# bioinfo-biols/CIRI-long

Hardware: AMD Instinct MI355X
Metric: reads/s through CCS+SSW+BSJ (1/2/4/8 MI355X); % HBM roofline (higher is better)
Workload: dtype int16

## Files before the change

ciri_long_amd/csrc/clh_api.hip:

```cpp
#include <hip/hip_runtime.h>
#include <stdint.h>
#include <stdio.h>
#include <stdlib.h>
#include <string.h>

#include <algorithm>
#include <chrono>
#include <mutex>
#include <string>
#include <vector>

#include "../../include/ciri_long_hip.h"
#include "../../include/ssw_legacy.h"
#include "clh_device.h"

static thread_local std::string g_err;
static thread_local int g_code = CLH_E_ARG;
static int fail(int code, const std::string& m) { g_err = m; g_code = code; return code; }
#define HIPCHK(expr)                                                                         \
    do {                                                                                     \
        hipError_t e_ = (expr);                                                              \
        if (e_ != hipSuccess) return fail(CLH_E_HIP, std::string(#expr) + ": " + hipGetErrorString(e_)); \
    } while (0)

// ... 110 lines not shown
    {
        (void)hipSetDevice(ctx->device);
        if (ran) (void)hipStreamSynchronize(last_stream);
        for (void* b : blocks) ctx->release(b);
        for (hipEvent_t e : events) (void)hipEventDestroy(e);
    }
    void* alloc(size_t bytes)
    {
        void* p = ctx->alloc(bytes);
        if (p) blocks.push_back(p);
        return p;
    }
    void* upload(const void* host, size_t bytes)
    {
        void* p = alloc(bytes);
        return p && (bytes == 0 || hipMemcpy(p, host, bytes, hipMemcpyHostToDevice) == hipSuccess) ? p : nullptr;
    }
    void free_block(void* p)
    {
        auto it = std::find(blocks.begin(), blocks.end(), p);
        if (it == blocks.end()) return;
        blocks.erase(it);
        ctx->release(p);
    }
    hipError_t event(hipEvent_t* e, unsigned flags = hipEventDefault)
    {
        const hipError_t r = hipEventCreateWithFlags(e, flags);
        if (r == hipSuccess) events.push_back(*e);
        return r;
    }
};

struct SswSwitches {
    bool no_scan, no_scanw, no_slices, no_prefilter, no_lanes, no_pf2, no_tb_rows, no_guess, pf2_always;
    int pf2_share;
};

static SswSwitches ssw_switches()
{
    SswSwitches sw;
    sw.no_scan = getenv("CLH_NO_SCAN") != nullptr;
    sw.no_scanw = getenv("CLH_NO_SCANW") != nullptr;
    sw.no_slices = getenv("CLH_NO_SLICES") != nullptr;
    sw.no_prefilter = getenv("CLH_NO_PREFILTER") != nullptr;
    sw.no_lanes = getenv("CLH_NO_LANES") != nullptr;
    sw.no_pf2 = getenv("CLH_NO_PF2") != nullptr;
    sw.no_tb_rows = getenv("CLH_NO_TB_ROWS") != nullptr;
    sw.no_guess = getenv("CLH_NO_GUESS") != nullptr;
    sw.pf2_always = getenv("CLH_PF2_ALWAYS") != nullptr;
    const char* share = getenv("CLH_PF2_SHARE");
    sw.pf2_share = share ? std::max(1, atoi(share)) : 8;
    return sw;
}

struct clh_plan : clh_owned {
    using clh_owned::clh_owned;
    int n = 0;
    clh_ssw_opts opts;
    SswSwitches sw;
    clh::SswParams params;
    bool quirk = false, do_cigar = false;
    std::vector<clh::SswTask> tasks;
    struct Seg { int rv, begin, count; int64_t ws_off = 0; int ws_slot = 0, ws_wgs = 0; int lmax = 0; };
    void* d_seg_ctr = nullptr;
    std::vector<clh::ScanSlice> slices;
    void *d_slices = nullptr, *d_parts = nullptr;
    struct PfClass {
        bool on = false;
        int ntasks = 0, nwork = 0, bpl = 0, cap = 0;
        void *d_win = nullptr, *d_pieces = nullptr, *d_work = nullptr, *d_dmin = nullptr, *d_queue = nullptr, *d_out = nullptr, *d_ctl = nullptr,
             *d_bound = nullptr, *d_parts = nullptr, *d_q2 = nullptr;
        int ws_row0 = 0, ws_slot = 0, ws_wgs = 0;
        int64_t ws_dirs_off = 0;
        int64_t extent = 0;
        int64_t word_cols = 0, lane_insts = 0;
        hipEvent_t ev[2] = {nullptr, nullptr};
        bool timed = false;
    } pf[2];
    int n_rows = 0;
    std::vector<int32_t> slice_base;
    void* d_slice_base = nullptr;
    int n_all = 0;
    std::vector<Seg> segs;
    void *d_tasks = nullptr, *d_results = nullptr, *d_colmax = nullptr, *d_cigars = nullptr, *d_cigar_len = nullptr,
         *d_pool = nullptr, *d_pool_head = nullptr;
    size_t colmax_elems = 0, cigar_elems = 0, strip_bytes = 0;
    unsigned long long pool_bytes = 0;
    void* d_strips = nullptr;
    hipEvent_t done_ev = nullptr;
    bool profiling = false;
    int64_t refs_bytes = -1;
    std::vector<hipEvent_t> ev;
    std::vector<int32_t> w32_prefix;
    bool alpha = false;
    void* d_alpha_mat = nullptr;
    const void *run_reads = nullptr, *run_refs = nullptr;

    int64_t reserve_ws(size_t bytes, int wgs, int* slot)
    {
        *slot = (int)((bytes + 255) & ~(size_t)255);
        strip_bytes = (strip_bytes + 255) & ~(size_t)255;
        const int64_t off = (int64_t)strip_bytes;
        strip_bytes += (size_t)*slot * (size_t)wgs;
        return off;
    }
};

extern "C" void clh_plan_destroy(clh_plan* pl) { delete pl; }

static int alpha_class_for(int64_t L)
{
    for (int b = 0; b < clh::kNumAlphaBuckets - 1; ++b)
        if (L <= clh::kAlphaRows[b]) return clh::kRvAlpha - b;
    return clh::kRvAlpha - (clh::kNumAlphaBuckets - 1);
}

static int rv_class_for(int64_t L)
{
    const int64_t rows = (L + 15) / 16 * 16;
    for (int i = 0; i < clh::kNumRvClasses; ++i)
        if (128 * clh::kRvClasses[i] >= rows) return clh::kRvClasses[i];
    return clh::kRvStrips;
}

static bool scan_class_ok(int64_t L, const clh_ssw_opts* o, int max_match, int bias, const SswSwitches& sw)
{
    return !sw.no_scan && L <= 254 && o->score_size != 1 && (int64_t)max_match * L + bias < 255 && o->gap_extend >= 0 && o->gap_extend <= 16 && o->gap_open <= 255;
}
// ... 262 lines not shown
    }
    for (const auto& sg : pl->segs) {
        if (sg.rv != clh::kRvScanSliced || pl->pf[0].on) continue;
        for (int k = 0; k < sg.count; ++k) {
            clh::SswTask& t = pl->tasks[sg.begin + k];
            const int64_t R = t.ref_len;
            const auto [overlap, own] = slice_geom(t.read_len, R, mx, o->gap_extend, 0);
            t.dir_off = (int64_t)pl->slices.size();
            int ns = 0;
            for (int64_t b = 0; b < R; b += own, ++ns) {
                clh::ScanSlice sl;
                memset(&sl, 0, sizeof(sl));
                sl.task = k; sl.own_begin = (int32_t)b; sl.c_begin = (int32_t)std::max<int64_t>(0, b - overlap); sl.c_end = (int32_t)std::min<int64_t>(R, b + own);
                sl.part = (int32_t)pl->slices.size();
                pl->slices.push_back(sl);
            }
            t.pad = ns;
        }
    }

    pl->d_tasks = n_all > 0 ? pl->upload(pl->tasks.data(), sizeof(clh::SswTask) * (size_t)n_all) : pl->alloc(sizeof(clh::SswTask));
    pl->d_results = pl->alloc(sizeof(clh::SswResult) * (size_t)std::max(pl->n_rows, 1));
    pl->d_cigar_len = pl->alloc(sizeof(int32_t) * (size_t)std::max(n_all, 1));
    if (!pl->d_tasks || !pl->d_results || !pl->d_cigar_len) return oom();
    if (!pl->slice_base.empty() && !(pl->d_slice_base = pl->upload(pl->slice_base.data(), sizeof(int32_t) * pl->slice_base.size()))) return oom();
    if (o->want_score2 && !(pl->d_colmax = pl->alloc(sizeof(uint16_t) * std::max<size_t>(colmax, 1)))) return oom();
    if (pl->do_cigar) {
        pl->d_cigars = pl->alloc(sizeof(uint32_t) * std::max<size_t>(cig, 1));
        pl->d_pool = pl->alloc((size_t)pl->pool_bytes);
        pl->d_pool_head = pl->alloc(clh::tb_head_bytes(n_all));
        if (!pl->d_cigars || !pl->d_pool || !pl->d_pool_head) return oom();
    }
    if (pl->strip_bytes && !(pl->d_strips = pl->alloc(pl->strip_bytes))) return oom();
    if (!pl->slices.empty()) {
        pl->d_slices = pl->upload(pl->slices.data(), sizeof(clh::ScanSlice) * pl->slices.size());
        pl->d_parts = pl->alloc(sizeof(clh::ScanPart) * pl->slices.size());
        if (!pl->d_slices || !pl->d_parts) return oom();
    }
    return pl;
}

extern "C" clh_plan* clh_ssw_plan(clh_ctx* ctx, int32_t n, const int64_t* read_off, const int64_t* ref_off,
                                  const int32_t* mask_len, const clh_ssw_opts* o)
{
    if (!ref_off) { fail(CLH_E_ARG, "clh_ssw_plan: null argument"); return nullptr; }
    return ssw_plan_build(ctx, n, read_off, ref_off, nullptr, nullptr, nullptr, mask_len, o);
}

extern "C" clh_plan* clh_ssw_plan_windows(clh_ctx* ctx, int32_t n, const int64_t* read_off, const int64_t* win_off, const int32_t* win_len,
                                          const uint8_t* win_rc, const int32_t* mask_len, const clh_ssw_opts* o)
{
    if (!win_off || !win_len) { fail(CLH_E_ARG, "clh_ssw_plan_windows: null argument"); return nullptr; }
    return ssw_plan_build(ctx, n, read_off, nullptr, win_off, win_len, win_rc, mask_len, o);
}

struct clh_genome : clh_owned {
    using clh_owned::clh_owned;
    int64_t len = 0;
    void *d_codes = nullptr, *d_pre = nullptr;
    void* d_ascii = nullptr;
    void* d_sites = nullptr;
    int64_t n_sites[4] = {0, 0, 0, 0};
};

extern "C" void clh_genome_destroy(clh_genome* g) { delete g; }

// ... 101 lines not shown
        t.ctg_off = ctg_off[i]; t.ctg_len = ctg_len[i]; t.start = start[i]; t.end = end[i]; t.clip_base = clip_base[i]; t.host_mask = host_mask[i];
    }
    clh_ctx* ctx = g->ctx;
    HIPCHK(hipSetDevice(ctx->device));
    const size_t tb = sizeof(clh::SpliceTask) * (size_t)n, ob = sizeof(int32_t) * 8 * (size_t)n;
    void* d_t = ctx->alloc(tb); void* d_o = ctx->alloc(ob);
    clh::SpliceSites sites;
    int64_t at = 0;
    for (int k = 0; k < 4; ++k) { sites.pos[k] = (const int64_t*)g->d_sites + at; sites.n[k] = g->n_sites[k]; at += g->n_sites[k]; }
    int rc = 0;
    if (!d_t || !d_o) rc = fail(CLH_E_HIP, "out of device memory");
    if (!rc && (hipMemcpyAsync(d_t, tasks.data(), tb, hipMemcpyHostToDevice, ctx->stream) != hipSuccess ||
                clh::launch_splice_scan((const uint8_t*)g->d_codes, (const uint8_t*)g->d_ascii, (const clh::SpliceTask*)d_t, n, search_extra, shift_threshold, is_canonical & 3,
                                        sites, (int32_t*)d_o, ctx->stream) != hipSuccess ||
                hipMemcpyAsync(out, d_o, ob, hipMemcpyDeviceToHost, ctx->stream) != hipSuccess ||
                hipStreamSynchronize(ctx->stream) != hipSuccess))
        rc = fail(CLH_E_HIP, "splice-signal scan failed");
    if (rc) (void)hipStreamSynchronize(ctx->stream);
    ctx->release(d_t); ctx->release(d_o);
    return rc;
}

extern "C" int clh_ssw_run(clh_plan* pl, const void* d_reads, const void* d_refs, void* stream_)
{
    if (!pl || !d_reads || !d_refs) return fail(CLH_E_ARG, "clh_ssw_run: null argument");
    HIPCHK(hipSetDevice(pl->ctx->device));
    hipStream_t st = stream_ ? (hipStream_t)stream_ : pl->ctx->stream;
    clh::SswParams P = pl->params;
    P.reads = (const int8_t*)d_reads; P.refs = (const int8_t*)d_refs;
    P.results = (clh::SswResult*)pl->d_results;
    P.colmax = (uint16_t*)pl->d_colmax;
    P.cigars = (uint32_t*)pl->d_cigars; P.cigar_len = (int32_t*)pl->d_cigar_len; P.dirs = (uint8_t*)pl->d_strips;
    P.no_guess = pl->sw.no_guess;
    pl->run_reads = d_reads; pl->run_refs = d_refs;
    if (pl->profiling && pl->ev.empty()) {
        pl->ev.resize(pl->segs.size() * 2 + 4);
        for (auto& e : pl->ev) HIPCHK(pl->event(&e));
    }
    clh_ctx* c = pl->ctx;
    const bool tb = pl->do_cigar && pl->n > 0;
    const bool fan = !pl->profiling && pl->segs.size() > 1;
    const size_t eb = pl->segs.size() * 2;
    if (tb) HIPCHK(hipMemsetAsync(pl->d_pool_head, 0, 4 * 68, st));
    if (fan) {
        HIPCHK(hipEventRecord(c->fork_ev, st));
        for (int i = 0; i < 3; ++i) HIPCHK(hipStreamWaitEvent(c->side[i], c->fork_ev, 0));
    }
    std::vector<size_t> ord(pl->segs.size());
    for (size_t k = 0; k < ord.size(); ++k) ord[k] = k;
    std::sort(ord.begin(), ord.end(), [&](size_t x, size_t y) {
        auto weight = [](int rv) { return rv == clh::kRvStrips ? 1000 : (rv == clh::kRvScanWide ? 900 : (rv == clh::kRvScanWideSliced ? 800 : (rv == clh::kRvScanTr ? 700 : (clh::rv_is_alpha(rv) ? 600 + clh::kRvAlpha - rv : rv)))); };
        const int rx = weight(pl->segs[x].rv), ry = weight(pl->segs[y].rv);
        return rx > ry;
    });
    clh::SswParams PG = P;
    PG.tasks = (const clh::SswTask*)pl->d_tasks;
    uint8_t* const pool = (uint8_t*)pl->d_pool;
    unsigned long long* const head = (unsigned long long*)pl->d_pool_head;
    auto traceback = [&](int first, int count, int seg, hipStream_t ls) -> int {
        const int rvbig = 32;
        if (!pl->sw.no_tb_rows) {
            HIPCHK(clh::launch_traceback_rows(PG, first, count, pl->n_all, seg, pool, head, pl->pool_bytes, ls));
            HIPCHK(clh::launch_traceback_rows_wide(PG, first, count, pl->n_all, seg, pool, head, pl->pool_bytes, ls));
        } else HIPCHK(clh::launch_traceback_pool(0, PG, first, count, pl->n_all, seg, pool, head, pl->pool_bytes, ls));
        HIPCHK(clh::launch_traceback_pool(rvbig, PG, first, count, pl->n_all, seg, pool, head, pl->pool_bytes, ls));
        if (pl->w32_prefix[first + count] > pl->w32_prefix[first]) HIPCHK(clh::launch_traceback_w32(PG, first, count, pool, head, pl->pool_bytes, ls));
// ... 138 lines not shown
    if (pl->do_cigar && pl->n > 0) {
        HIPCHK(hipEventElapsedTime(&k1b_ms[0], pl->ev[2 * ns + 0], pl->ev[2 * ns + 1]));
        HIPCHK(hipEventElapsedTime(&k1b_ms[1], pl->ev[2 * ns + 2], pl->ev[2 * ns + 3]));
    }
    return ns;
}

extern "C" int clh_plan_traceback_counts(clh_plan* pl, int32_t* counts)
{
    if (!pl || !counts || !pl->ran) return fail(CLH_E_ARG, "clh_plan_traceback_counts: no run yet");
    counts[0] = counts[1] = 0;
    if (!pl->d_pool_head) return 0;
    HIPCHK(hipSetDevice(pl->ctx->device));
    HIPCHK(hipStreamSynchronize(pl->last_stream));
    int32_t w[64];
    HIPCHK(hipMemcpy(w, (const char*)pl->d_pool_head + 16, sizeof(w), hipMemcpyDeviceToHost));
    for (int k = 0; k < 32; ++k) { counts[0] += w[k]; counts[1] += w[32 + k]; }
    return 0;
}

extern "C" int clh_plan_prefilter_stats(clh_plan* pl, int64_t* out)
{
    if (!pl || !out) return fail(CLH_E_ARG, "clh_plan_prefilter_stats: null argument");
    for (int k = 0; k < 6; ++k) out[k] = 0;
    if (!pl->ran) return 0;
    HIPCHK(hipSetDevice(pl->ctx->device));
    HIPCHK(hipStreamSynchronize(pl->last_stream));
    for (const auto& f : pl->pf) {
        if (!f.on) continue;
        clh::PfCtl c;
        HIPCHK(hipMemcpy(&c, f.d_ctl, sizeof(c), hipMemcpyDeviceToHost));
        out[0] += f.ntasks; out[1] += c.n_pruned; out[2] += c.qcount; out[3] += (int64_t)c.cols_scanned; out[4] += (int64_t)c.cols_window; out[5] += c.n_stage2;
    }
    return 0;
}

extern "C" int clh_plan_prefilter_timing(clh_plan* pl, float* ms, int64_t* work)
{
    if (!pl || !ms || !work) return fail(CLH_E_ARG, "clh_plan_prefilter_timing: null argument");
    if (!pl->ran || !pl->profiling) return fail(CLH_E_ARG, "profiling was not enabled for the last run");
    HIPCHK(hipSetDevice(pl->ctx->device));
    HIPCHK(hipStreamSynchronize(pl->last_stream));
    for (int ci = 0; ci < 2; ++ci) {
        const auto& f = pl->pf[ci];
        ms[ci] = 0.f; work[2 * ci] = work[2 * ci + 1] = 0;
        if (!f.on || !f.timed) continue;
        HIPCHK(hipEventElapsedTime(&ms[ci], f.ev[0], f.ev[1]));
        work[2 * ci] = f.word_cols; work[2 * ci + 1] = f.lane_insts;
    }
    return 0;
}

extern "C" const void* clh_ssw_results_dev(const clh_plan* pl) { return pl ? pl->d_results : nullptr; }

__global__ void cigar_gather_kernel(const uint32_t* __restrict__ src, const int32_t* __restrict__ src_off, const int64_t* __restrict__ dst_off,
                                    const int32_t* __restrict__ len, uint32_t* __restrict__ dst)
{
    const int a = blockIdx.x, L = len[a];
    const uint32_t* s = src + src_off[a];
    uint32_t* d = dst + dst_off[a];
    for (int k = threadIdx.x; k < L; k += blockDim.x) d[k] = s[k];
}

static int alpha_pool_rounds(clh_plan* pl, std::vector<clh::SswResult>& res)
{
    const int n = pl->n;
// ... 1285 lines not shown
```

ciri_long_amd/csrc/clh_device.h:

```cpp
#pragma once
#include <hip/hip_runtime.h>
#include <stdint.h>

namespace clh {

enum {
    CLH_STATUS_WORD = 1,
    CLH_STATUS_OVERFLOW8 = 2,
    CLH_STATUS_TRACE_ERR = 4,
    CLH_STATUS_NO_CIGAR = 8,
    CLH_STATUS_CIGAR_TRUNC = 16,
    CLH_STATUS_NEED_BIG = 32,
    CLH_STATUS_BAD_CODE = 64,
    CLH_STATUS_NEED_W32 = 128,
    CLH_STATUS_NEED_POOL = 256
};

struct SswTask {
    int64_t read_off;
    int64_t ref_off;
    int64_t colmax_off;
    int64_t dir_off;
    int32_t read_len;
    int32_t ref_len;
// ... 56 lines not shown
struct SswParams {
    const int8_t* reads;
    const int8_t* refs;
    const SswTask* tasks;
    SswResult* results;
    uint16_t* colmax;
    uint32_t* cigars;
    int32_t* cigar_len;
    uint8_t* dirs;
    int8_t mat[32];
    int32_t n, gapO, gapE, bias, max_match, score_size, flag, filters, filterd;
    int32_t null_code;
    const ScanSlice* slices;
    ScanPart* parts;
    int32_t n_real;
    const int32_t* slice_base;
    const PfWin* pf_win;
    const PfTask* pf_tasks;
    const PfWork* pf_work;
    uint8_t* pf_dmin;
    ScanSlice* pf_slices;
    PfOut* pf_out;
    PfCtl* pf_ctl;
    int32_t pf_bpl, pf_cap;
    int32_t* pf_q2;
    int32_t pf2_always;
    int32_t pf2_share;
    uint16_t* ws_bound;
    WsTask* ws_tasks;
    int32_t ws_row0;
    int32_t ws_slot_bytes;
    int64_t ws_dirs_off;
    int32_t no_guess;
};

static constexpr int CCS_SEG_CAP = 65;

struct CcsScan {
    int32_t period;
    int32_t ncuts;
    int32_t support;
    int32_t cuts[64];
};

struct CcsResult {
    int32_t nseg;
    int32_t ccs_len;
    int32_t period;
    int32_t status;
};

struct PoaScores {
    int32_t algorithm;
    int32_t m, n, g, e, q, c;
    int32_t min_cov;
};

struct CcsParams {
    const int8_t* reads;
    const int64_t* read_off;
    CcsScan* scan;
    CcsResult* results;
    int32_t* segs;
    int8_t* ccs;
    uint8_t* poa_ws;
    int* work_counter;
// ... 168 lines not shown
```

ciri_long_amd/csrc/ssw_scan.hip:

```cpp
#include <hip/hip_runtime.h>
#include <stdint.h>
#include "clh_device.h"
#include "clh_device_ops.h"

namespace clh {

namespace {



#ifndef SCAN_WAVES
#define SCAN_WAVES 3
#endif
static constexpr int SCAN_MAX_ROWS = 256;
static constexpr int SCAN_CPR_MAX = 8;
static constexpr int SCAN_PROF_WORDS = 6 * SCAN_CPR_MAX * 64;

struct ScanIn {
    const int8_t* read;
    int rstep;
    int L;
    int rows;
    const int8_t* ref;
    int cstep;
    int comp;
    int ncols;
    int terminate;
    uint16_t* colmax;
    int own0;
    int col_base;
};
struct ScanOut { int max, col, row; };

struct ScanLds {
    uint32_t* prof;
    const int* mat;
    short* bH;
    short* bE;
};

template <int CPR, bool GEQ>
__device__ void scan_chunk(const ScanIn& in, const ScanLds& lds, const int c0, const int parity, const bool first, const bool more,
                           const int gapO, const int gapE, int& best_score, int& best_col, int& best_row, int& tcol)
{
    constexpr int VEC = CPR < 4 ? CPR : 4;
    constexpr int NCH = CPR / VEC;
    const int lane = threadIdx.x & 63;
    const int K = CPR * gapE;
    const int kLo = 2 * lane * K;
    const uint32_t gO2 = dup16(gapO), gE2 = dup16(gapE);

    {
        int rlo[CPR], rhi[CPR];
#pragma unroll
        for (int t = 0; t < CPR; ++t) {
            const int jlo = c0 + 2 * CPR * lane + t, jhi = jlo + CPR;
            const int blo = jlo < in.ncols ? (int)in.ref[(int64_t)jlo * in.cstep] : 0, bhi = jhi < in.ncols ? (int)in.ref[(int64_t)jhi * in.cstep] : 0;
            rlo[t] = jlo < in.ncols ? ref_code(blo, in.comp) : 5;
            rhi[t] = jhi < in.ncols ? ref_code(bhi, in.comp) : 5;
        }
#pragma unroll
        for (int q = 0; q < 6; ++q)
#pragma unroll
            for (int t = 0; t < CPR; ++t) {
                const int slo = lds.mat[rlo[t] * 8 + q], shi = lds.mat[rhi[t] * 8 + q];
                lds.prof[((q * NCH + t / VEC) * 64 + lane) * VEC + (t % VEC)] = (uint32_t)(slo & 0xffff) | ((uint32_t)shi << 16);
            }
    }
    const short* bHin = lds.bH + (parity ^ 1) * SCAN_MAX_ROWS;
    const short* bEin = lds.bE + (parity ^ 1) * SCAN_MAX_ROWS;
    short* bHout = lds.bH + parity * SCAN_MAX_ROWS;
// ... 136 lines not shown
    res.score1 = fw.max;
    if (fw.max == 0) { res.ref_end1 = -1; res.read_end1 = 0; }
    else { res.ref_end1 = fw.col; res.read_end1 = fw.row; }
    if (task.mask_len >= 15 && colmax) { __syncthreads(); __builtin_amdgcn_fence(__ATOMIC_ACQUIRE, "agent"); second_best(colmax, refLen, res.ref_end1, task.mask_len, 0, res.score2, res.ref_end2); }
    else { res.score2 = 0; res.ref_end2 = task.mask_len >= 15 ? 0 : -1; }

    res.read_begin1 = -1;
    const bool want_begin = !(p.flag == 0 || (p.flag == 2 && res.score1 < p.filters));
    if (want_begin) {
        ScanIn rv;
        rv.L = res.read_end1 + 1; rv.rows = ((rv.L + 15) / 16) * 16; rv.read = read + res.read_end1; rv.rstep = -1;
        rv.ncols = res.ref_end1 + 1; rv.ref = ref + (int64_t)res.ref_end1 * rdir; rv.cstep = -rdir; rv.comp = task.ref_rc;
        rv.terminate = res.score1; rv.colmax = nullptr; rv.own0 = 0; rv.col_base = 0;
        const ScanOut r = scan_pass<GEQ>(rv, lds, p.gapO, p.gapE);
        if (r.max == 0) { res.ref_begin1 = -1; res.read_begin1 = res.read_end1; }
        else { res.ref_begin1 = res.ref_end1 - r.col; res.read_begin1 = res.read_end1 - r.row; }
    }
    if (lane == 0) p.results[task.out_index] = res;
}

template <bool GEQ>
__device__ ScanOut scan_forward(const SswParams& p, const SswTask& task, const ScanLds& lds, int c_begin, int own_begin, int c_end)
{
    const int rdir = task.ref_rc ? -1 : 1;
    uint16_t* colmax = p.colmax ? p.colmax + task.colmax_off : nullptr;
    ScanIn in;
    in.read = p.reads + task.read_off; in.rstep = 1; in.L = task.read_len;
    in.ref = p.refs + task.ref_off + (int64_t)c_begin * rdir; in.cstep = rdir; in.comp = task.ref_rc; in.ncols = c_end - c_begin;
    in.terminate = 1 << 30; in.colmax = colmax; in.own0 = own_begin - c_begin; in.col_base = c_begin;
    in.rows = colmax ? ((in.L + 15) / 16) * 16 : in.L;
    return scan_pass<GEQ>(in, lds, p.gapO, p.gapE);
}

#define SCAN_LDS_SETUP \
    __shared__ __attribute__((aligned(16))) uint32_t s_prof[SCAN_PROF_WORDS]; \
    __shared__ int s_mat[48]; \
    __shared__ short s_bH[2 * SCAN_MAX_ROWS], s_bE[2 * SCAN_MAX_ROWS]; \
    { const int lane_ = threadIdx.x & 63; \
      if (lane_ < 48) { const int b_ = lane_ >> 3, q_ = lane_ & 7; s_mat[lane_] = (b_ < p.n && q_ < p.n) ? (int)p.mat[b_ * p.n + q_] : 0; } } \
    __syncthreads(); \
    ScanLds lds; lds.prof = s_prof; lds.mat = s_mat; lds.bH = s_bH; lds.bE = s_bE;

}

template <bool GEQ>
__global__ void __launch_bounds__(64, SCAN_WAVES) ssw_scan_kernel(const SswParams p)
{
    SCAN_LDS_SETUP
    const SswTask task = p.tasks[blockIdx.x];
    const ScanOut fw = scan_forward<GEQ>(p, task, lds, 0, 0, task.ref_len);
    scan_finish<GEQ>(p, task, fw, lds);
}

template <bool GEQ>
__global__ void __launch_bounds__(64, SCAN_WAVES) ssw_scan_slice_kernel(const SswParams p)
{
    SCAN_LDS_SETUP
    const ScanSlice sl = p.slices[blockIdx.x];
    const SswTask task = p.tasks[sl.task];
    const ScanOut fw = scan_forward<GEQ>(p, task, lds, sl.c_begin, sl.own_begin, sl.c_end);
    if ((threadIdx.x & 63) == 0) { ScanPart pt; pt.max = fw.max; pt.col = fw.col; pt.row = fw.row; pt.pad = 0; p.parts[sl.part] = pt; }
}

template <bool GEQ>
__global__ void __launch_bounds__(64, SCAN_WAVES) ssw_scan_finish_kernel(const SswParams p)
{
    SCAN_LDS_SETUP
    const int lane = threadIdx.x & 63;
    const SswTask task = p.tasks[blockIdx.x];
    const int first = (int)task.dir_off, ns = task.pad;
    int v = 0, c = 0x7fffffff, r = 0;
    if (lane < ns) { const ScanPart pt = p.parts[first + lane]; v = pt.max; c = pt.max > 0 ? pt.col : 0x7fffffff; r = pt.row; }
#pragma unroll
    for (int d = 1; d < 64; d <<= 1) {
        const int v2 = __shfl_xor(v, d), c2 = __shfl_xor(c, d), r2 = __shfl_xor(r, d);
        const bool take = v2 > v || (v2 == v && c2 < c);
        v = take ? v2 : v; c = take ? c2 : c; r = take ? r2 : r;
    }
    ScanOut fw; fw.max = v; fw.col = v > 0 ? c : -1; fw.row = v > 0 ? r : 0;
    scan_finish<GEQ>(p, task, fw, lds);
}

template <bool GEQ>
// ... 249 lines not shown
```

ciri_long_amd/hip.py:

```python
import ctypes as C
import os
import sys

import numpy as np

_HERE = os.path.dirname(os.path.abspath(__file__))
SO_PATH = os.environ.get('CLH_LIB') or os.path.join(_HERE, 'libclh.so')


class HipUnavailable(RuntimeError):
    pass


class ClhError(RuntimeError):
    pass


class AlignRow(C.Structure):
    _fields_ = [('score1', C.c_uint16), ('score2', C.c_uint16), ('ref_begin1', C.c_int32), ('ref_end1', C.c_int32),
                ('read_begin1', C.c_int32), ('read_end1', C.c_int32), ('ref_end2', C.c_int32),
                ('cigar_off', C.c_int32), ('cigar_len', C.c_int32), ('status', C.c_int32)]


ALIGN_DTYPE = np.dtype([('score1', '<u2'), ('score2', '<u2'), ('ref_begin1', '<i4'), ('ref_end1', '<i4'),
# ... 92 lines not shown
        L.clh_edit_distance_batch.restype = C.c_int
        L.clh_edit_matrix_plan_create.restype = C.c_void_p
        L.clh_edit_matrix_plan_create.argtypes = [C.c_void_p, C.c_int32, C.c_void_p, C.c_void_p, C.c_int32, C.c_void_p, C.c_int32]
        L.clh_edit_matrix_plan_destroy.restype = None
        L.clh_edit_matrix_plan_destroy.argtypes = [C.c_void_p]
        L.clh_edit_matrix_plan_run.argtypes = [C.c_void_p, C.c_void_p]
        L.clh_edit_matrix_plan_sizes.argtypes = [C.c_void_p, C.POINTER(C.c_int64), C.POINTER(C.c_int64)]
        L.clh_edit_matrix_plan_fetch.argtypes = [C.c_void_p, C.c_void_p, C.c_int64, C.c_void_p, C.c_void_p, C.c_int64]
        L.clh_edit_matrix_plan_timing.argtypes = [C.c_void_p, C.c_void_p]
        L.clh_edit_matrix_batch.argtypes = [C.c_void_p, C.c_int32, C.c_void_p, C.c_void_p, C.c_int32, C.c_void_p, C.c_int32, C.c_void_p, C.c_int64,
                                            C.c_void_p, C.c_void_p, C.c_int64]
        L.clh_edit_align_plan_create.restype = C.c_void_p
        L.clh_edit_align_plan_create.argtypes = [C.c_void_p, C.c_int32, C.c_void_p, C.c_void_p, C.c_void_p, C.c_void_p, C.POINTER(EditAlignOpts)]
        L.clh_edit_align_plan_destroy.restype = None
        L.clh_edit_align_plan_destroy.argtypes = [C.c_void_p]
        L.clh_edit_align_plan_run.argtypes = [C.c_void_p, C.c_void_p]
        L.clh_edit_align_plan_fetch.argtypes = [C.c_void_p, C.c_void_p, C.c_void_p, C.c_int64, C.POINTER(C.c_int64), C.c_void_p, C.c_int64,
                                                C.POINTER(C.c_int64)]
        L.clh_edit_align_plan_timing.argtypes = [C.c_void_p, C.c_void_p]
        L.clh_edit_align_plan_caps.argtypes = [C.c_void_p, C.POINTER(C.c_int64), C.POINTER(C.c_int64)]
        L.clh_edit_align_batch.argtypes = [C.c_void_p, C.c_int32, C.c_void_p, C.c_void_p, C.c_void_p, C.c_void_p, C.POINTER(EditAlignOpts),
                                           C.c_void_p, C.c_void_p, C.c_int64, C.POINTER(C.c_int64), C.c_void_p, C.c_int64, C.POINTER(C.c_int64)]
        L.clh_poa_batch.argtypes = [C.c_void_p, C.c_int32, C.c_void_p, C.c_void_p, C.c_void_p, C.c_void_p, C.c_void_p, C.c_void_p,
                                    C.c_void_p, C.c_void_p, C.c_void_p]
        L.clh_ccs_results_dev.argtypes = [C.c_void_p, C.c_void_p, C.c_void_p, C.c_void_p]
        L.clh_ccs_plan_info.argtypes = [C.c_void_p, C.c_void_p]
        L.clh_ccs_plan_stats.argtypes = [C.c_void_p, C.c_void_p]
        L.clh_poa_last_stats.argtypes = [C.c_void_p, C.c_void_p]
        L.clh_plan_set_profiling.argtypes = [C.c_void_p, C.c_int]
        L.clh_plan_segments.argtypes = [C.c_void_p, C.c_int32, C.c_void_p, C.c_void_p, C.c_void_p, C.c_void_p]
        L.clh_plan_timing.argtypes = [C.c_void_p, C.c_int32, C.c_void_p, C.c_void_p]
        L.clh_plan_traceback_counts.argtypes = [C.c_void_p, C.c_void_p]
        L.clh_plan_prefilter_stats.argtypes = [C.c_void_p, C.c_void_p]
        L.clh_plan_prefilter_timing.argtypes = [C.c_void_p, C.c_void_p, C.c_void_p]
        L.clh_plan_set_refs_bytes.argtypes = [C.c_void_p, C.c_int64]
        _lib = L
    return _lib


def fastx_index(in_path, is_fastq, every=4096):
    n = C.c_int64(0); no = C.c_int64(0)
    L = lib()
    L.clh_fastx_index.argtypes = [C.c_char_p, C.c_int, C.c_int64, C.c_void_p, C.c_void_p, C.c_int64, C.c_void_p]
    cap = max(16, os.path.getsize(in_path) // max(1, 20 * every) + 16)
    off = np.zeros(cap, dtype=np.int64)
    if L.clh_fastx_index(os.fsencode(in_path), int(bool(is_fastq)), int(every), C.byref(n), off.ctypes.data, cap, C.byref(no)) != 0:
        raise ClhError('clh_fastx_index failed for %s' % in_path)
    return int(n.value), [int(x) for x in off[:no.value]]


def fastx_count(in_path, is_fastq):
    n = C.c_int64(0)
    if lib().clh_fastx_count(os.fsencode(in_path), int(bool(is_fastq)), C.byref(n)) != 0:
        raise ClhError('clh_fastx_count failed for %s' % in_path)
    return int(n.value)


def last_error():
    return lib().clh_last_error().decode()


def _check(rc, what):
    if rc != 0:
        raise ClhError('%s failed (%d): %s' % (what, rc, last_error()))


# ... 534 lines not shown
    def run(self, d_reads_ptr, d_refs_ptr, stream=0):
        _check(lib().clh_ssw_run(self._h, C.c_void_p(d_reads_ptr), C.c_void_p(d_refs_ptr), C.c_void_p(stream)), 'clh_ssw_run')

    def fetch(self):
        out = np.zeros(self.n, dtype=ALIGN_DTYPE)
        cap = int(2 * (self.read_off[-1] if self.n else 0) + 2 * self.n + 8) if self.want_cigar else 1
        cig = np.empty(cap, dtype=np.uint32)
        used = C.c_int64(0)
        _check(lib().clh_ssw_fetch(self._h, out.ctypes.data, cig.ctypes.data if self.want_cigar else None, cap, C.byref(used)), 'clh_ssw_fetch')
        return out, cig[:used.value]

    def set_refs_bytes(self, nbytes):
        lib().clh_plan_set_refs_bytes(self._h, int(nbytes))

    def set_profiling(self, on=True):
        lib().clh_plan_set_profiling(self._h, 1 if on else 0)

    def segments(self):
        rv = np.zeros(32, dtype=np.int32); cnt = np.zeros(32, dtype=np.int32)
        rb = np.zeros(32, dtype=np.int64); fb = np.zeros(32, dtype=np.int64)
        ns = lib().clh_plan_segments(self._h, 32, rv.ctypes.data, cnt.ctypes.data, rb.ctypes.data, fb.ctypes.data)
        return [(int(rv[k]), int(cnt[k]), int(rb[k]), int(fb[k])) for k in range(ns)]

    def traceback_counts(self):
        c = np.zeros(2, dtype=np.int32)
        _check(lib().clh_plan_traceback_counts(self._h, c.ctypes.data), 'clh_plan_traceback_counts')
        return int(c[0]), int(c[1])

    def prefilter_stats(self):
        c = np.zeros(6, dtype=np.int64)
        _check(lib().clh_plan_prefilter_stats(self._h, c.ctypes.data), 'clh_plan_prefilter_stats')
        return dict(zip(('alignments', 'pruned', 'slices', 'cols_computed', 'cols_window', 'second_stage'), (int(x) for x in c)))

    def prefilter_timing(self):
        ms = np.zeros(2, dtype=np.float32); w = np.zeros(4, dtype=np.int64)
        _check(lib().clh_plan_prefilter_timing(self._h, ms.ctypes.data, w.ctypes.data), 'clh_plan_prefilter_timing')
        return [(float(ms[k]), int(w[2 * k]), int(w[2 * k + 1])) for k in range(2)]

    def timing(self):
        a = np.zeros(32, dtype=np.float32); b = np.zeros(2, dtype=np.float32)
        ns = lib().clh_plan_timing(self._h, 32, a.ctypes.data, b.ctypes.data)
        if ns < 0:
            _check(ns, 'clh_plan_timing')
        return [float(a[k]) for k in range(ns)], (float(b[0]), float(b[1]))

    def results_dev_ptr(self):
        return lib().clh_ssw_results_dev(self._h)


class CcsPlan(_Handle):
    _destroy = 'clh_ccs_plan_destroy'

    def __init__(self, ctx, read_off):
        _Handle.__init__(self, ctx)
        self.read_off = np.ascontiguousarray(read_off, dtype=np.int64)
        self.n = len(self.read_off) - 1
        self._h = lib().clh_ccs_plan_create(ctx._h, self.n, self.read_off.ctypes.data)
        if not self._h:
            raise ClhError('clh_ccs_plan_create failed: %s' % last_error())

    def run(self, d_reads_ptr, stream=0):
        _check(lib().clh_ccs_run(self._h, C.c_void_p(d_reads_ptr), C.c_void_p(stream)), 'clh_ccs_run')

    def timing(self):
        ms = np.zeros(2, dtype=np.float32)
        _check(lib().clh_ccs_plan_timing(self._h, ms.ctypes.data), 'clh_ccs_plan_timing')
# ... 35 lines not shown
```

include/ciri_long_hip.h:

```cpp
#ifndef CIRI_LONG_HIP_H
#define CIRI_LONG_HIP_H

#include <stdint.h>

#ifdef __cplusplus
extern "C" {
#endif
#pragma GCC visibility push(default)

#define CLH_E_HIP        (-1)
#define CLH_E_ARG        (-2)
#define CLH_E_UNSUPPORTED (-3)
#define CLH_E_CAPACITY   (-4)

#define CLH_ST_WORD        1
#define CLH_ST_NULL        2
#define CLH_ST_TRACE_ERR   4
#define CLH_ST_NO_CIGAR    8
#define CLH_ST_CIGAR_TRUNC 16

typedef struct {
    uint16_t score1;
    uint16_t score2;
    int32_t ref_begin1;
// ... 7 lines not shown
} clh_align_t;

typedef struct clh_ctx clh_ctx;
typedef struct clh_plan clh_plan;

int clh_device_count(void);
const char* clh_last_error(void);
const char* clh_version(void);

clh_ctx* clh_create(int device);
void clh_destroy(clh_ctx* ctx);
int clh_device_of(const clh_ctx* ctx);

typedef struct {
    const int8_t* mat;
    int32_t n_mat;
    uint8_t gap_open;
    uint8_t gap_extend;
    uint8_t flag;
    int8_t score_size;
    uint16_t filters;
    int32_t filterd;
    int32_t want_score2;
    int32_t want_cigar;
} clh_ssw_opts;

clh_plan* clh_ssw_plan(clh_ctx* ctx, int32_t n, const int64_t* read_off, const int64_t* ref_off,
                       const int32_t* mask_len, const clh_ssw_opts* opts);
void clh_plan_destroy(clh_plan* plan);

int clh_plan_traceback_counts(clh_plan* pl, int32_t* counts);

int clh_plan_prefilter_stats(clh_plan* pl, int64_t* out);

int clh_plan_prefilter_timing(clh_plan* pl, float* ms, int64_t* work);

int clh_ssw_run(clh_plan* plan, const void* d_reads, const void* d_refs, void* stream);

int clh_plan_set_refs_bytes(clh_plan* plan, int64_t nbytes);

int clh_ssw_fetch(clh_plan* plan, clh_align_t* out, uint32_t* cigar_buf, int64_t cigar_cap, int64_t* cigar_used);

const void* clh_ssw_results_dev(const clh_plan* plan);

int clh_plan_set_profiling(clh_plan* plan, int on);
int clh_plan_segments(const clh_plan* plan, int32_t cap, int32_t* rv, int32_t* count, int64_t* read_bases, int64_t* ref_bases);
int clh_plan_timing(clh_plan* plan, int32_t cap, float* k1_ms, float* k1b_ms);

int clh_ssw_batch(clh_ctx* ctx, int32_t n, const int8_t* reads, const int64_t* read_off, const int8_t* refs,
                  const int64_t* ref_off, const int32_t* mask_len, const clh_ssw_opts* opts,
                  clh_align_t* out, uint32_t* cigar_buf, int64_t cigar_cap, int64_t* cigar_used);

#define CLH_CCS_SEG_CAP 65
typedef struct {
    int32_t nseg;
    int32_t ccs_len;
    int32_t period;
    int32_t status;
} clh_ccs_t;
typedef struct clh_ccs_plan clh_ccs_plan;
clh_ccs_plan* clh_ccs_plan_create(clh_ctx* ctx, int32_t n, const int64_t* read_off);
void clh_ccs_plan_destroy(clh_ccs_plan* plan);
int clh_ccs_run(clh_ccs_plan* plan, const void* d_reads, void* stream);
int clh_ccs_fetch(clh_ccs_plan* plan, clh_ccs_t* out, int32_t* segs, int8_t* ccs);
int clh_ccs_results_dev(const clh_ccs_plan* plan, const void** rows, const void** segs, const void** ccs);
int clh_ccs_plan_info(clh_ccs_plan* plan, int64_t* out);
// ... 89 lines not shown
```

Baseline: 5.235 million.

## Prune SSW scan columns with bit-parallel edit-distance lower bounds

```diff
diff --git a/ciri_long_amd/csrc/clh_api.hip b/ciri_long_amd/csrc/clh_api.hip
--- a/ciri_long_amd/csrc/clh_api.hip
+++ b/ciri_long_amd/csrc/clh_api.hip
@@ -166,8 +166,8 @@
 };
 
 struct SswSwitches {
-    bool no_scan, no_scanw, no_slices, no_prefilter, no_lanes, no_pf2, no_tb_rows, no_guess, pf2_always;
-    int pf2_share;
+    bool no_scan, no_scanw, no_slices, no_prefilter, no_lanes, no_pf2, no_tb_rows, no_guess, pf2_always, no_scan_prune;
+    int pf2_share, scan_prune_mult, scan_prune_share;
 };
 
 static SswSwitches ssw_switches()
@@ -184,6 +184,11 @@
     sw.pf2_always = getenv("CLH_PF2_ALWAYS") != nullptr;
     const char* share = getenv("CLH_PF2_SHARE");
     sw.pf2_share = share ? std::max(1, atoi(share)) : 8;
+    sw.no_scan_prune = getenv("CLH_NO_SCAN_PRUNE") != nullptr;
+    const char* mult = getenv("CLH_SCAN_PRUNE_MULT");
+    sw.scan_prune_mult = mult ? std::max(1, atoi(mult)) : 4;
+    const char* pshare = getenv("CLH_SCAN_PRUNE_SHARE");
+    sw.scan_prune_share = pshare ? std::min(100, std::max(0, atoi(pshare))) : 50;
     return sw;
 }
 
@@ -228,6 +233,7 @@
     std::vector<int32_t> w32_prefix;
     bool alpha = false;
     void* d_alpha_mat = nullptr;
+    void* d_scan_prune = nullptr;
     const void *run_reads = nullptr, *run_refs = nullptr;
 
     int64_t reserve_ws(size_t bytes, int wgs, int* slot)
@@ -556,6 +562,11 @@
         if (!pl->d_cigars || !pl->d_pool || !pl->d_pool_head) return oom();
     }
     if (pl->strip_bytes && !(pl->d_strips = pl->alloc(pl->strip_bytes))) return oom();
+    if (!alpha && !sw.no_scan_prune && prefilter_ok(o, mx, sw) &&
+        std::any_of(pl->segs.begin(), pl->segs.end(), [](const clh_plan::Seg& g) { return g.rv == clh::kRvScan; })) {
+        const unsigned long long zero[3] = {0, 0, 0};
+        if (!(pl->d_scan_prune = pl->upload(zero, sizeof(zero)))) return oom();
+    }
     if (!pl->slices.empty()) {
         pl->d_slices = pl->upload(pl->slices.data(), sizeof(clh::ScanSlice) * pl->slices.size());
         pl->d_parts = pl->alloc(sizeof(clh::ScanPart) * pl->slices.size());
@@ -723,6 +734,8 @@
     P.colmax = (uint16_t*)pl->d_colmax;
     P.cigars = (uint32_t*)pl->d_cigars; P.cigar_len = (int32_t*)pl->d_cigar_len; P.dirs = (uint8_t*)pl->d_strips;
     P.no_guess = pl->sw.no_guess;
+    P.scan_prune_ctr = (unsigned long long*)pl->d_scan_prune;
+    P.scan_prune = pl->d_scan_prune != nullptr; P.scan_prune_mult = pl->sw.scan_prune_mult; P.scan_prune_share = pl->sw.scan_prune_share;
     pl->run_reads = d_reads; pl->run_refs = d_refs;
     if (pl->profiling && pl->ev.empty()) {
         pl->ev.resize(pl->segs.size() * 2 + 4);
@@ -927,6 +940,17 @@
         HIPCHK(hipMemcpy(&c, f.d_ctl, sizeof(c), hipMemcpyDeviceToHost));
         out[0] += f.ntasks; out[1] += c.n_pruned; out[2] += c.qcount; out[3] += (int64_t)c.cols_scanned; out[4] += (int64_t)c.cols_window; out[5] += c.n_stage2;
     }
+    return 0;
+}
+
+extern "C" int clh_plan_scan_prune_stats(clh_plan* pl, int64_t* out)
+{
+    if (!pl || !out) return fail(CLH_E_ARG, "clh_plan_scan_prune_stats: null argument");
+    for (int k = 0; k < 3; ++k) out[k] = 0;
+    if (!pl->d_scan_prune) return 0;
+    HIPCHK(hipSetDevice(pl->ctx->device));
+    if (pl->ran) HIPCHK(hipStreamSynchronize(pl->last_stream));
+    HIPCHK(hipMemcpy(out, pl->d_scan_prune, 3 * sizeof(int64_t), hipMemcpyDeviceToHost));
     return 0;
 }
 
diff --git a/ciri_long_amd/csrc/clh_device.h b/ciri_long_amd/csrc/clh_device.h
--- a/ciri_long_amd/csrc/clh_device.h
+++ b/ciri_long_amd/csrc/clh_device.h
@@ -112,6 +112,10 @@
     int32_t ws_slot_bytes;
     int64_t ws_dirs_off;
     int32_t no_guess;
+    int32_t scan_prune;
+    int32_t scan_prune_mult;
+    int32_t scan_prune_share;
+    unsigned long long* scan_prune_ctr;
 };
 
 static constexpr int CCS_SEG_CAP = 65;
diff --git a/ciri_long_amd/csrc/ssw_scan.hip b/ciri_long_amd/csrc/ssw_scan.hip
--- a/ciri_long_amd/csrc/ssw_scan.hip
+++ b/ciri_long_amd/csrc/ssw_scan.hip
@@ -37,6 +37,7 @@
     const int* mat;
     short* bH;
     short* bE;
+    uint32_t* lmin;
 };
 
 template <int CPR, bool GEQ>
@@ -239,14 +240,147 @@
     return scan_pass<GEQ>(in, lds, p.gapO, p.gapE);
 }
 
+__device__ __forceinline__ int wave_prefix_sum(int v)
+{
+    const int lane = threadIdx.x & 63;
+#pragma unroll
+    for (int d = 1; d < 64; d <<= 1) { const int o = __shfl_up(v, d); v += lane >= d ? o : 0; }
+    return v;
+}
+
+template <int W>
+__device__ __forceinline__ uint32_t prune_distances(const SswParams& p, const SswTask& task, const ScanLds& lds)
+{
+    const int lane = threadIdx.x & 63;
+    const int R = task.ref_len, L = task.read_len;
+    const int rdir = task.ref_rc ? -1 : 1;
+    const int8_t* ref = p.refs + task.ref_off;
+    const int8_t* read = p.reads + task.read_off;
+    const int cc = p.max_match < p.gapE ? p.max_match : p.gapE;
+    uint32_t eqt;
+    { const int b = lane / 5, q = lane - 5 * b; eqt = (uint32_t)__ballot(lane < 30 && lds.mat[b * 8 + q] > p.max_match - cc); }
+    uint32_t* eqL = lds.prof;
+#pragma unroll
+    for (int w = 0; w < W; ++w) {
+        uint32_t e[5] = {0, 0, 0, 0, 0};
+        const int col0 = 32 * (64 * w + lane);
+#pragma unroll 8
+        for (int b = 0; b < 32; ++b) {
+            const int j = col0 + b;
+            int code = 5;
+            if (j < R) code = ref_code((int)ref[(int64_t)j * rdir], task.ref_rc);
+            const uint32_t t = (eqt >> (5 * code)) & 31u;
+#pragma unroll
+            for (int q = 0; q < 5; ++q) e[q] = __builtin_amdgcn_alignbit(t >> q, e[q], 1);
+        }
+#pragma unroll
+        for (int q = 0; q < 5; ++q) eqL[(q * W + w) * 64 + lane] = e[q];
+        eqL[(5 * W + w) * 64 + lane] = 0;
+    }
+    __syncthreads();
+
+    uint32_t Pv[W], Mv[W];
+#pragma unroll
+    for (int w = 0; w < W; ++w) { Pv[w] = 0; Mv[w] = 0; }
+    for (int rb = 0; rb < L; rb += 64) {
+        const int row = rb + lane;
+        int qv = 5;
+        if (row < L) { const int c = (int)read[row] & 7; qv = c > 5 ? 5 : c; }
+        const int cnt = L - rb < 64 ? L - rb : 64;
+        for (int i = 0; i < cnt; ++i) {
+            const int q = __builtin_amdgcn_readlane(qv, i);
+            const uint32_t* eqr = eqL + q * W * 64 + lane;
+            unsigned long long cin = 0;
+            int fillP = (int)0x80000000u, fillM = 0;
+#pragma unroll
+            for (int w = 0; w < W; ++w) {
+                const uint32_t Eq = eqr[w * 64];
+                const uint32_t Xv = Eq | Mv[w];
+                const uint32_t a = Eq & Pv[w];
+                uint32_t sum = a + Pv[w];
+                const unsigned long long G = __ballot(sum < a), Pm = __ballot(sum == 0xffffffffu);
+                const unsigned long long x = G | Pm, s1 = x + G, s2 = s1 + cin;
+                if (w + 1 < W) cin = (unsigned long long)((s1 < x) | (s2 < s1));
+                sum += (uint32_t)(((s2 ^ Pm) >> lane) & 1ull);
+                const uint32_t Xh = (sum ^ Pv[w]) | Eq;
+                const uint32_t Ph = Mv[w] | ~(Xh | Pv[w]);
+                const uint32_t Mh = Pv[w] & Xh;
+                const uint32_t Phs = __builtin_amdgcn_alignbit(Ph, (uint32_t)dpp_shr1(fillP, (int)Ph), 31);
+                const uint32_t Mhs = __builtin_amdgcn_alignbit(Mh, (uint32_t)dpp_shr1(fillM, (int)Mh), 31);
+                if (w + 1 < W) { fillP = __builtin_amdgcn_readlane((int)Ph, 63); fillM = __builtin_amdgcn_readlane((int)Mh, 63); }
+                Pv[w] = Mhs | ~(Xv | Phs);
+                Mv[w] = Phs & Xv;
+            }
+        }
+    }
+    uint32_t pk = 0;
+    int before = L;
+#pragma unroll
+    for (int w = 0; w < W; ++w) {
+        const int delta = __popc(Pv[w]) - __popc(Mv[w]);
+        const int incl = wave_prefix_sum(delta);
+        int d = before + incl - delta;
+        before += __builtin_amdgcn_readlane(incl, 63);
+        int nv = R - 32 * (64 * w + lane);
+        nv = nv > 32 ? 32 : nv;
+        int mn = 255;
+#pragma unroll
+        for (int b = 0; b < 32; ++b) {
+            d += (int)((Pv[w] >> b) & 1u) - (int)((Mv[w] >> b) & 1u);
+            const int m2 = d < mn ? d : mn;
+            mn = b < nv ? m2 : mn;
+        }
+        pk |= (uint32_t)mn << (8 * w);
+    }
+    __syncthreads();
+    return pk;
+}
+
+__device__ __forceinline__ unsigned long long prune_word(const unsigned long long (&m)[4], int w)
+{
+    return w == 0 ? m[0] : (w == 1 ? m[1] : (w == 2 ? m[2] : m[3]));
+}
+__device__ __forceinline__ bool prune_next_set_run(const unsigned long long (&m)[4], int pos, int& gs, int& ge)
+{
+    int g = pos;
+    bool found = false;
+    while (g < 256) {
+        const unsigned long long v = prune_word(m, g >> 6) >> (g & 63);
+        if (v) { g += __builtin_ctzll(v); found = true; break; }
+        g = (g | 63) + 1;
+    }
+    if (!found) return false;
+    gs = g;
+    while (g < 256) {
+        const unsigned long long v = ~(prune_word(m, g >> 6) >> (g & 63));
+        const int z = v ? __builtin_ctzll(v) : 64;
+        g += z;
+        if (z == 0 || (g & 63) != 0) break;
+    }
+    ge = g;
+    return true;
+}
+__device__ __forceinline__ bool prune_next_run(const unsigned long long (&m)[4], int& pos, int overlap, int& gs, int& ge)
+{
+    if (!prune_next_set_run(m, pos, gs, ge)) return false;
+    for (;;) {
+        int gs2, ge2;
+        if (!prune_next_set_run(m, ge, gs2, ge2) || 32 * (gs2 - ge) >= overlap) break;
+        ge = ge2;
+    }
+    pos = ge;
+    return true;
+}
+
 #define SCAN_LDS_SETUP \
     __shared__ __attribute__((aligned(16))) uint32_t s_prof[SCAN_PROF_WORDS]; \
     __shared__ int s_mat[48]; \
     __shared__ short s_bH[2 * SCAN_MAX_ROWS], s_bE[2 * SCAN_MAX_ROWS]; \
+    __shared__ uint32_t s_lmin[64]; \
     { const int lane_ = threadIdx.x & 63; \
       if (lane_ < 48) { const int b_ = lane_ >> 3, q_ = lane_ & 7; s_mat[lane_] = (b_ < p.n && q_ < p.n) ? (int)p.mat[b_ * p.n + q_] : 0; } } \
     __syncthreads(); \
-    ScanLds lds; lds.prof = s_prof; lds.mat = s_mat; lds.bH = s_bH; lds.bE = s_bE;
+    ScanLds lds; lds.prof = s_prof; lds.mat = s_mat; lds.bH = s_bH; lds.bE = s_bE; lds.lmin = s_lmin;
 
 }
 
@@ -254,8 +388,58 @@
 __global__ void __launch_bounds__(64, SCAN_WAVES) ssw_scan_kernel(const SswParams p)
 {
     SCAN_LDS_SETUP
+    const int lane = threadIdx.x & 63;
     const SswTask task = p.tasks[blockIdx.x];
-    const ScanOut fw = scan_forward<GEQ>(p, task, lds, 0, 0, task.ref_len);
+    const int R = task.ref_len, L = task.read_len;
+    enum { kFull, kSeed, kRuns };
+    int mode = kFull, cb = 0, ob = 0, ce = R;
+    int overlap = 0, thr = 0, cols = 0;
+    bool fell_back = false;
+    if (p.scan_prune && L >= 1 && R <= 8192) {
+        overlap = L + (L * p.max_match + p.gapE - 1) / p.gapE + 32;
+        if (R < p.scan_prune_mult * overlap) overlap = 0;
+    }
+    if (overlap) {
+        const uint32_t pk = R <= 2048 ? prune_distances<1>(p, task, lds) : (R <= 4096 ? prune_distances<2>(p, task, lds) : prune_distances<4>(p, task, lds));
+        lds.lmin[lane] = pk;
+        int key = 0x7fffffff;
+#pragma unroll
+        for (int w = 0; w < 4; ++w) { const int v = (int)(((pk >> (8 * w)) & 255u) << 8) | (64 * w + lane); key = (32 * (64 * w + lane) < R && v < key) ? v : key; }
+        const int seed_g = __builtin_amdgcn_readfirstlane(wave_min(key)) & 255;
+        mode = kSeed; ob = 32 * seed_g; ce = ob + 32 > R ? R : ob + 32; cb = ob - overlap < 0 ? 0 : ob - overlap;
+    }
+    ScanOut fw; fw.max = 0; fw.col = -1; fw.row = 0;
+    for (;;) {
+        ScanOut r = scan_forward<GEQ>(p, task, lds, cb, ob, ce);
+        r.max = __builtin_amdgcn_readfirstlane(r.max); r.col = __builtin_amdgcn_readfirstlane(r.col); r.row = __builtin_amdgcn_readfirstlane(r.row);
+        cols += ce - cb;
+        if (mode == kFull) { fw = r; break; }
+        int pos = (ce + 31) >> 5;
+        if (mode == kSeed) {
+            fell_back = r.max == 0;
+            const int cc = p.max_match < p.gapE ? p.max_match : p.gapE;
+            thr = (p.max_match * L - r.max) / cc;
+            pos = 0;
+        } else if (r.max > fw.max) fw = r;
+        unsigned long long m[4];
+        {
+            const uint32_t pk = lds.lmin[lane];
+#pragma unroll
+            for (int w = 0; w < 4; ++w) m[w] = __ballot((int)((pk >> (8 * w)) & 255u) <= thr && 32 * (64 * w + lane) < R);
+        }
+        int gs, ge;
+        if (mode == kSeed && !fell_back) {
+            if (__popcll(m[0]) + __popcll(m[1]) + __popcll(m[2]) + __popcll(m[3]) == 1) { fw = r; break; }
+            int cost = 0, q = 0;
+            while (prune_next_run(m, q, overlap, gs, ge)) cost += (32 * ge > R ? R : 32 * ge) - (32 * gs - overlap < 0 ? 0 : 32 * gs - overlap);
+            fell_back = 100 * (long long)cost > (long long)p.scan_prune_share * R;
+        }
+        if (fell_back) { mode = kFull; cb = 0; ob = 0; ce = R; continue; }
+        mode = kRuns;
+        if (!prune_next_run(m, pos, overlap, gs, ge)) break;
+        ob = 32 * gs; ce = 32 * ge > R ? R : 32 * ge; cb = ob - overlap < 0 ? 0 : ob - overlap;
+    }
+    if (overlap && lane < 3) atomicAdd(&p.scan_prune_ctr[lane], lane == 0 ? (unsigned long long)!fell_back : (lane == 1 ? (unsigned long long)fell_back : (unsigned long long)cols));
     scan_finish<GEQ>(p, task, fw, lds);
 }
 
diff --git a/ciri_long_amd/hip.py b/ciri_long_amd/hip.py
--- a/ciri_long_amd/hip.py
+++ b/ciri_long_amd/hip.py
@@ -148,6 +148,8 @@
         L.clh_plan_timing.argtypes = [C.c_void_p, C.c_int32, C.c_void_p, C.c_void_p]
         L.clh_plan_traceback_counts.argtypes = [C.c_void_p, C.c_void_p]
         L.clh_plan_prefilter_stats.argtypes = [C.c_void_p, C.c_void_p]
+        if hasattr(L, 'clh_plan_scan_prune_stats'):
+            L.clh_plan_scan_prune_stats.argtypes = [C.c_void_p, C.c_void_p]
         L.clh_plan_prefilter_timing.argtypes = [C.c_void_p, C.c_void_p, C.c_void_p]
         L.clh_plan_set_refs_bytes.argtypes = [C.c_void_p, C.c_int64]
         _lib = L
@@ -748,6 +750,11 @@
         _check(lib().clh_plan_prefilter_stats(self._h, c.ctypes.data), 'clh_plan_prefilter_stats')
         return dict(zip(('alignments', 'pruned', 'slices', 'cols_computed', 'cols_window', 'second_stage'), (int(x) for x in c)))
 
+    def scan_prune_stats(self):
+        c = np.zeros(3, dtype=np.int64)
+        _check(lib().clh_plan_scan_prune_stats(self._h, c.ctypes.data), 'clh_plan_scan_prune_stats')
+        return dict(zip(('pruned', 'fell_back', 'cols_computed'), (int(x) for x in c)))
+
     def prefilter_timing(self):
         ms = np.zeros(2, dtype=np.float32); w = np.zeros(4, dtype=np.int64)
         _check(lib().clh_plan_prefilter_timing(self._h, ms.ctypes.data, w.ctypes.data), 'clh_plan_prefilter_timing')
diff --git a/include/ciri_long_hip.h b/include/ciri_long_hip.h
--- a/include/ciri_long_hip.h
+++ b/include/ciri_long_hip.h
@@ -63,6 +63,8 @@
 int clh_plan_traceback_counts(clh_plan* pl, int32_t* counts);
 
 int clh_plan_prefilter_stats(clh_plan* pl, int64_t* out);
+
+int clh_plan_scan_prune_stats(clh_plan* pl, int64_t* out);
 
 int clh_plan_prefilter_timing(clh_plan* pl, float* ms, int64_t* work);
 
```

New measurement: 5.379 million, median of 5. 1.03x the previous value.
